# althonos/nafcodec

Measured on AMD Instinct MI355X. Metric: decoded Gbases/s (+ GB/s off HBM) at 1/2/4/8 MI355X vs CPU ref, higher is better.
Workload: dtype u8; 1 GPU; synthetic 10.0 GB DNA-only .naf (seq+len), 40000000000 bases, 73052 records, 152588 zstd blocks / 610352 Huffman streams in all, zstd-level-1 shape (L1), full-size check against the WRITER's checksums of bases and record table skipped

## Files before the change

nafcodec_amd/csrc/huf_flat.hip:

```cpp
#include <hip/hip_runtime.h>

#include <cstdlib>

#include "kernels.h"
#include "plan.h"

namespace nafgpu {

namespace {

#ifdef NAFGPU_EMU
#define NAFGPU_FLAT_INLINE inline
#else
#define NAFGPU_FLAT_INLINE __forceinline__
#endif

constexpr uint32_t kFlatThreads = 256;
constexpr uint32_t kFlatUnroll = 4;

__device__ inline void flat_flag_error(uint32_t *status, uint32_t code, uint32_t detail) {
    if (atomicCAS(&status[0], 0u, code) == 0u) status[1] = detail;
}

__device__ inline uint32_t flat_nib_char(uint32_t nib, uint32_t t_char) {
    const uint64_t lo = 0x425359434B47002Dull | (static_cast<uint64_t>(t_char) << 8);
    const uint64_t hi = 0x4E56484D44525741ull;
    return static_cast<uint32_t>(((nib & 8u) ? hi : lo) >> (8u * (nib & 7u))) & 0xFFu;
}
__device__ inline uint32_t flat_byte_chars(uint32_t b, uint32_t t_char) {
    return flat_nib_char(b & 15u, t_char) | (flat_nib_char(b >> 4, t_char) << 8);
}

template <bool ASCII, uint32_t L>
__device__ NAFGPU_FLAT_INLINE void flat_stream(const uint8_t *sp, uint32_t n, uint8_t *dp, const uint16_t *__restrict__ x1, uint32_t t_char,
                                   uint32_t *s_tbl) {
    constexpr uint32_t kOutB = ASCII ? 2 : 1;
    constexpr uint32_t kSyms = 16 / kOutB;
    constexpr uint32_t kPer = L <= 4 ? 2 : 1;
    constexpr uint32_t kIdxBits = kPer * L;
    constexpr uint32_t kLookB = kPer * kOutB;
    constexpr uint32_t kWords = (kSyms * L + 31) / 32;
    constexpr uint32_t kCodeMask = (1u << L) - 1u;
    const uint32_t tid = threadIdx.x;

    for (uint32_t i = tid; i < (1u << kIdxBits); i += kFlatThreads) {
        const uint32_t s1 = x1[kPer == 2 ? i >> L : i] & 0xFFu, s2 = x1[i & kCodeMask] & 0xFFu;
        const uint32_t o1 = ASCII ? flat_byte_chars(s1, t_char) : s1, o2 = ASCII ? flat_byte_chars(s2, t_char) : s2;
        s_tbl[i] = kPer == 2 ? o1 | (o2 << (8 * kOutB)) : o1;
    }
    __syncthreads();

    const uint32_t h = static_cast<uint32_t>(reinterpret_cast<uintptr_t>(dp) & 15u);
    uint8_t *const d16 = dp - h;
    const uintptr_t sa = reinterpret_cast<uintptr_t>(sp);
    const uint32_t *const sw = reinterpret_cast<const uint32_t *>(sp - (sa & 3u));
    const uint32_t sbit = static_cast<uint32_t>(sa & 3u) * 8u;
    const uint32_t end = h + n * kOutB;
    const uint32_t pf0 = h ? 1u : 0u, pf1 = end >> 4;
    constexpr uint32_t kStepWords = kFlatThreads * kSyms * L / 32u;
    uint32_t first = pf0 + tid;
    uint32_t r = 0;
    const uint32_t *w0 = sw;
    if (first < pf1) {
        const uint32_t lo = (n - (first * 16u - h) / kOutB - kSyms) * L + sbit;
        r = lo & 31u;
        w0 = sw + (lo >> 5);
    }
    auto load_round = [&](uint32_t p0, const uint32_t *w, uint32_t (&raw)[kFlatUnroll][kWords + 1]) {
#pragma unroll
        for (uint32_t u = 0; u < kFlatUnroll; u++) {
            const uint32_t *wu = p0 + u * kFlatThreads < pf1 ? w - u * kStepWords : w;
#pragma unroll
            for (uint32_t k = 0; k <= kWords; k++) raw[u][k] = wu[k];
        }
    };
    uint32_t cur[kFlatUnroll][kWords + 1];
    if (first < pf1) load_round(first, w0, cur);
    while (first < pf1) {
        const uint32_t next = first + kFlatUnroll * kFlatThreads;
        const uint32_t *w1 = w0 - kFlatUnroll * kStepWords;
        uint32_t nxt[kFlatUnroll][kWords + 1];
        if (next < pf1) load_round(next, w1, nxt);
#pragma unroll
        for (uint32_t u = 0; u < kFlatUnroll; u++) {
            const uint32_t p = first + u * kFlatThreads;
            uint32_t nw[kWords];
#pragma unroll
            for (uint32_t k = 0; k < kWords; k++) nw[k] = __builtin_amdgcn_alignbit(cur[u][k + 1], cur[u][k], r);
            uint32_t o[4] = {0, 0, 0, 0};
#pragma unroll
            for (uint32_t t = 0; t < kSyms / kPer; t++) {
                const uint32_t off = (kSyms - kPer * (t + 1u)) * L, q = off >> 5, s = off & 31u;
                uint32_t v = nw[q] >> s;
                if (s + kIdxBits > 32u) v |= nw[q + 1] << (32u - s);
                const uint32_t e = s_tbl[v & ((1u << kIdxBits) - 1u)];
                o[(t * kLookB) >> 2] |= e << (8u * ((t * kLookB) & 3u));
            }
            if (p < pf1) *reinterpret_cast<uint4 *>(d16 + static_cast<size_t>(p) * 16u) = make_uint4(o[0], o[1], o[2], o[3]);
        }
        if (next < pf1) {
#pragma unroll
            for (uint32_t u = 0; u < kFlatUnroll; u++)
#pragma unroll
                for (uint32_t k = 0; k <= kWords; k++) cur[u][k] = nxt[u][k];
        }
        first = next;
        w0 = w1;
    }
    const bool tail = (end & 15u) != 0 && (pf1 != 0 || !h);
    if ((tid == 0 && h) || (tid == 1 && tail)) {
        const uint32_t p = tid == 0 ? 0u : pf1;
        const int32_t j0 = (static_cast<int32_t>(p * 16u) - static_cast<int32_t>(h)) / static_cast<int32_t>(kOutB);
        for (uint32_t i = 0; i < kSyms; i++) {
            const int32_t j = j0 + static_cast<int32_t>(i);
            if (j < 0 || static_cast<uint32_t>(j) >= n) continue;
            const uint32_t b = (n - 1u - static_cast<uint32_t>(j)) * L;
            uint32_t v = sp[b >> 3];
            if ((b & 7u) + L > 8u) v |= static_cast<uint32_t>(sp[(b >> 3) + 1u]) << 8;
            const uint32_t code = (v >> (b & 7u)) & kCodeMask;
            const uint32_t e = s_tbl[kPer == 2 ? code << L : code];
            uint8_t *d = dp + static_cast<size_t>(j) * kOutB;
            d[0] = static_cast<uint8_t>(e);
            if (ASCII) d[1] = static_cast<uint8_t>(e >> 8);
        }
    }
}

template <bool ASCII>
__global__ __launch_bounds__(256) void k_huf_flat(const uint8_t *__restrict__ src, const HufTask *__restrict__ tasks,
                                                  const HufTblCopy *__restrict__ copies, const HufStream *__restrict__ streams,
                                                  const uint16_t *__restrict__ pool, const uint64_t *__restrict__ blk_base,
                                                  uint8_t *dst_base, uint32_t t_char, uint32_t *status) {
    constexpr uint32_t kOutB = ASCII ? 2 : 1;
    __shared__ uint32_t s_tbl[256];
    if (status[0] != 0) return;
    const HufTask task = tasks[blockIdx.x / static_cast<uint32_t>(kHufWave)];
    const uint32_t k = blockIdx.x % static_cast<uint32_t>(kHufWave);
    if (k >= task.n_streams) return;
    const uint32_t me = task.first_stream + k;
    const HufStream st = streams[me];
    const uint32_t L = st.max_bits;
    const uint32_t lastb = src[st.src_end - 1];
    const uint32_t hb = 31u - static_cast<uint32_t>(__clz(static_cast<int>(lastb | 1u)));
    const uint64_t bits = static_cast<uint64_t>(st.src_len - 1u) * 8u + hb;
    if (lastb == 0 || bits != static_cast<uint64_t>(st.n_syms) * L) {
        if (threadIdx.x == 0) flat_flag_error(status, kStHufBadEnd, me);
        return;
    }
    const uint8_t *sp = src + (st.src_end - st.src_len);
    uint8_t *dp = dst_base + ((st.flags & 1u) ? st.dst : (blk_base[st.blk] + static_cast<uint32_t>(st.dst)) * kOutB);
    const uint16_t *x1 = pool + copies[task.first_copy + st.tbl_lds].pool_off;
    switch (L) {
    case 1: flat_stream<ASCII, 1>(sp, st.n_syms, dp, x1, t_char, s_tbl); break;
    case 2: flat_stream<ASCII, 2>(sp, st.n_syms, dp, x1, t_char, s_tbl); break;
    case 3: flat_stream<ASCII, 3>(sp, st.n_syms, dp, x1, t_char, s_tbl); break;
    case 4: flat_stream<ASCII, 4>(sp, st.n_syms, dp, x1, t_char, s_tbl); break;
    case 5: flat_stream<ASCII, 5>(sp, st.n_syms, dp, x1, t_char, s_tbl); break;
    case 6: flat_stream<ASCII, 6>(sp, st.n_syms, dp, x1, t_char, s_tbl); break;
    case 7: flat_stream<ASCII, 7>(sp, st.n_syms, dp, x1, t_char, s_tbl); break;
    case 8: flat_stream<ASCII, 8>(sp, st.n_syms, dp, x1, t_char, s_tbl); break;
    default:
        if (threadIdx.x == 0) flat_flag_error(status, kStInternal, me);
        break;
    }
}

}

void launch_huf_flat(hipStream_t stream, const uint8_t *src, const HufTask *tasks, const HufClass &cls, const HufTblCopy *copies,
                     const HufStream *streams, const uint16_t *pool, const uint64_t *blk_base, uint8_t *out, uint8_t *lit,
                     bool ascii, uint32_t t_char, uint32_t *status) {
    if (!cls.n_tasks) return;
    const HufTask *t0 = tasks + cls.first_task;
    const dim3 grid(cls.n_tasks * static_cast<uint32_t>(kHufWave));
    if (ascii && !cls.to_lit)
        hipLaunchKernelGGL(k_huf_flat<true>, grid, dim3(kFlatThreads), 0, stream, src, t0, copies, streams, pool, blk_base, out, t_char, status);
    else
        hipLaunchKernelGGL(k_huf_flat<false>, grid, dim3(kFlatThreads), 0, stream, src, t0, copies, streams, pool, blk_base,
                           cls.to_lit ? lit : out, t_char, status);
}

}
```

Measured before the change: 4292 Gbases/s.

## Software-pipeline flat Huffman decode with ping-pong register rounds and early loads

Restructures the flat Huffman stream loop. Full rounds now run as unguarded double-buffered pairs: the next round's words are loaded while the current one is decoded and stored. Compiler barriers pin the load/store order, and the table staging into LDS is deferred until after the first loads are issued, so it overlaps with their latency. The kernel also hoists the status, pool-offset and block-base loads together and adds an occupancy hint to launch bounds. This trades extra register pressure and more code for better memory-latency hiding, with a guarded tail loop handling the remainder.

```diff
diff --git a/nafcodec_amd/csrc/huf_flat.hip b/nafcodec_amd/csrc/huf_flat.hip
--- a/nafcodec_amd/csrc/huf_flat.hip
+++ b/nafcodec_amd/csrc/huf_flat.hip
@@ -17,6 +17,8 @@
 
 constexpr uint32_t kFlatThreads = 256;
 constexpr uint32_t kFlatUnroll = 4;
+
+__device__ inline void flat_order() { asm volatile("" ::: "memory"); }
 
 __device__ inline void flat_flag_error(uint32_t *status, uint32_t code, uint32_t detail) {
     if (atomicCAS(&status[0], 0u, code) == 0u) status[1] = detail;
@@ -43,12 +45,14 @@
     constexpr uint32_t kCodeMask = (1u << L) - 1u;
     const uint32_t tid = threadIdx.x;
 
-    for (uint32_t i = tid; i < (1u << kIdxBits); i += kFlatThreads) {
-        const uint32_t s1 = x1[kPer == 2 ? i >> L : i] & 0xFFu, s2 = x1[i & kCodeMask] & 0xFFu;
-        const uint32_t o1 = ASCII ? flat_byte_chars(s1, t_char) : s1, o2 = ASCII ? flat_byte_chars(s2, t_char) : s2;
-        s_tbl[i] = kPer == 2 ? o1 | (o2 << (8 * kOutB)) : o1;
-    }
-    __syncthreads();
+    auto stage = [&]() {
+        for (uint32_t i = tid; i < (1u << kIdxBits); i += kFlatThreads) {
+            const uint32_t s1 = x1[kPer == 2 ? i >> L : i] & 0xFFu, s2 = x1[i & kCodeMask] & 0xFFu;
+            const uint32_t o1 = ASCII ? flat_byte_chars(s1, t_char) : s1, o2 = ASCII ? flat_byte_chars(s2, t_char) : s2;
+            s_tbl[i] = kPer == 2 ? o1 | (o2 << (8 * kOutB)) : o1;
+        }
+        __syncthreads();
+    };
 
     const uint32_t h = static_cast<uint32_t>(reinterpret_cast<uintptr_t>(dp) & 15u);
     uint8_t *const d16 = dp - h;
@@ -58,54 +62,85 @@
     const uint32_t end = h + n * kOutB;
     const uint32_t pf0 = h ? 1u : 0u, pf1 = end >> 4;
     constexpr uint32_t kStepWords = kFlatThreads * kSyms * L / 32u;
+    constexpr uint32_t kRound = kFlatUnroll * kFlatThreads;
     uint32_t first = pf0 + tid;
     uint32_t r = 0;
-    const uint32_t *w0 = sw;
+    uint32_t w0 = 0;
     if (first < pf1) {
         const uint32_t lo = (n - (first * 16u - h) / kOutB - kSyms) * L + sbit;
         r = lo & 31u;
-        w0 = sw + (lo >> 5);
-    }
-    auto load_round = [&](uint32_t p0, const uint32_t *w, uint32_t (&raw)[kFlatUnroll][kWords + 1]) {
-#pragma unroll
-        for (uint32_t u = 0; u < kFlatUnroll; u++) {
-            const uint32_t *wu = p0 + u * kFlatThreads < pf1 ? w - u * kStepWords : w;
+        w0 = lo >> 5;
+    }
+    auto words = [&](uint32_t w) { return reinterpret_cast<const uint32_t *>(reinterpret_cast<const uint8_t *>(sw) + w * 4u); };
+    auto piece = [&](uint32_t p) { return reinterpret_cast<uint4 *>(d16 + p * 16u); };
+    using Raw = uint32_t[kFlatUnroll][kWords + 1];
+    auto decode = [&](const uint32_t (&raw)[kWords + 1]) {
+        uint32_t nw[kWords];
+#pragma unroll
+        for (uint32_t k = 0; k < kWords; k++) nw[k] = __builtin_amdgcn_alignbit(raw[k + 1], raw[k], r);
+        uint32_t o[4] = {0, 0, 0, 0};
+#pragma unroll
+        for (uint32_t t = 0; t < kSyms / kPer; t++) {
+            const uint32_t off = (kSyms - kPer * (t + 1u)) * L, q = off >> 5, s = off & 31u;
+            uint32_t v = nw[q] >> s;
+            if (s + kIdxBits > 32u) v |= nw[q + 1] << (32u - s);
+            const uint32_t e = s_tbl[v & ((1u << kIdxBits) - 1u)];
+            o[(t * kLookB) >> 2] |= e << (8u * ((t * kLookB) & 3u));
+        }
+        return make_uint4(o[0], o[1], o[2], o[3]);
+    };
+    auto load_whole = [&](uint32_t w, Raw &raw) {
+#pragma unroll
+        for (uint32_t u = 0; u < kFlatUnroll; u++) {
+            const uint32_t *wu = words(w - u * kStepWords);
 #pragma unroll
             for (uint32_t k = 0; k <= kWords; k++) raw[u][k] = wu[k];
         }
-    };
-    uint32_t cur[kFlatUnroll][kWords + 1];
-    if (first < pf1) load_round(first, w0, cur);
-    while (first < pf1) {
-        const uint32_t next = first + kFlatUnroll * kFlatThreads;
-        const uint32_t *w1 = w0 - kFlatUnroll * kStepWords;
-        uint32_t nxt[kFlatUnroll][kWords + 1];
-        if (next < pf1) load_round(next, w1, nxt);
+        flat_order();
+    };
+    auto store_whole = [&](uint32_t p0, const Raw &raw) {
+#pragma unroll
+        for (uint32_t u = 0; u < kFlatUnroll; u++) {
+            *piece(p0 + u * kFlatThreads) = decode(raw[u]);
+            flat_order();
+        }
+    };
+    const uint32_t pairs = pf1 > pf0 ? (pf1 - pf0) / (2u * kRound) : 0u;
+    constexpr uint32_t kRoundWords = kFlatUnroll * kStepWords;
+    if (pairs) {
+        Raw a, b;
+        load_whole(w0, a);
+        load_whole(w0 - kRoundWords, b);
+        stage();
+        store_whole(first, a);
+        for (uint32_t i = 1; i < pairs; i++) {
+            load_whole(w0 - 2 * kRoundWords, a);
+            store_whole(first + kRound, b);
+            load_whole(w0 - 3 * kRoundWords, b);
+            store_whole(first + 2 * kRound, a);
+            first += 2 * kRound;
+            w0 -= 2 * kRoundWords;
+        }
+        store_whole(first + kRound, b);
+        first += 2 * kRound;
+        w0 -= 2 * kRoundWords;
+    } else {
+        stage();
+    }
+    for (; first < pf1; first += kRound, w0 -= kRoundWords) {
+        Raw c;
+#pragma unroll
+        for (uint32_t u = 0; u < kFlatUnroll; u++) {
+            const uint32_t *wu = words(first + u * kFlatThreads < pf1 ? w0 - u * kStepWords : w0);
+#pragma unroll
+            for (uint32_t k = 0; k <= kWords; k++) c[u][k] = wu[k];
+        }
 #pragma unroll
         for (uint32_t u = 0; u < kFlatUnroll; u++) {
             const uint32_t p = first + u * kFlatThreads;
-            uint32_t nw[kWords];
-#pragma unroll
-            for (uint32_t k = 0; k < kWords; k++) nw[k] = __builtin_amdgcn_alignbit(cur[u][k + 1], cur[u][k], r);
-            uint32_t o[4] = {0, 0, 0, 0};
-#pragma unroll
-            for (uint32_t t = 0; t < kSyms / kPer; t++) {
-                const uint32_t off = (kSyms - kPer * (t + 1u)) * L, q = off >> 5, s = off & 31u;
-                uint32_t v = nw[q] >> s;
-                if (s + kIdxBits > 32u) v |= nw[q + 1] << (32u - s);
-                const uint32_t e = s_tbl[v & ((1u << kIdxBits) - 1u)];
-                o[(t * kLookB) >> 2] |= e << (8u * ((t * kLookB) & 3u));
-            }
-            if (p < pf1) *reinterpret_cast<uint4 *>(d16 + static_cast<size_t>(p) * 16u) = make_uint4(o[0], o[1], o[2], o[3]);
-        }
-        if (next < pf1) {
-#pragma unroll
-            for (uint32_t u = 0; u < kFlatUnroll; u++)
-#pragma unroll
-                for (uint32_t k = 0; k <= kWords; k++) cur[u][k] = nxt[u][k];
-        }
-        first = next;
-        w0 = w1;
+            const uint4 o = decode(c[u]);
+            if (p < pf1) *piece(p) = o;
+        }
     }
     const bool tail = (end & 15u) != 0 && (pf1 != 0 || !h);
     if ((tid == 0 && h) || (tid == 1 && tail)) {
@@ -127,20 +162,24 @@
 }
 
 template <bool ASCII>
-__global__ __launch_bounds__(256) void k_huf_flat(const uint8_t *__restrict__ src, const HufTask *__restrict__ tasks,
+__global__ __launch_bounds__(256, ASCII ? 8 : 7) void k_huf_flat(const uint8_t *__restrict__ src, const HufTask *__restrict__ tasks,
                                                   const HufTblCopy *__restrict__ copies, const HufStream *__restrict__ streams,
                                                   const uint16_t *__restrict__ pool, const uint64_t *__restrict__ blk_base,
                                                   uint8_t *dst_base, uint32_t t_char, uint32_t *status) {
     constexpr uint32_t kOutB = ASCII ? 2 : 1;
     __shared__ uint32_t s_tbl[256];
-    if (status[0] != 0) return;
+    const uint32_t stopped = status[0];
     const HufTask task = tasks[blockIdx.x / static_cast<uint32_t>(kHufWave)];
     const uint32_t k = blockIdx.x % static_cast<uint32_t>(kHufWave);
-    if (k >= task.n_streams) return;
+    if (stopped != 0 || k >= task.n_streams) return;
     const uint32_t me = task.first_stream + k;
     const HufStream st = streams[me];
+    flat_order();
     const uint32_t L = st.max_bits;
     const uint32_t lastb = src[st.src_end - 1];
+    const uint32_t pool_off = copies[task.first_copy + st.tbl_lds].pool_off;
+    const uint64_t base = blk_base[st.blk];
+    flat_order();
     const uint32_t hb = 31u - static_cast<uint32_t>(__clz(static_cast<int>(lastb | 1u)));
     const uint64_t bits = static_cast<uint64_t>(st.src_len - 1u) * 8u + hb;
     if (lastb == 0 || bits != static_cast<uint64_t>(st.n_syms) * L) {
@@ -148,8 +187,8 @@
         return;
     }
     const uint8_t *sp = src + (st.src_end - st.src_len);
-    uint8_t *dp = dst_base + ((st.flags & 1u) ? st.dst : (blk_base[st.blk] + static_cast<uint32_t>(st.dst)) * kOutB);
-    const uint16_t *x1 = pool + copies[task.first_copy + st.tbl_lds].pool_off;
+    uint8_t *dp = dst_base + ((st.flags & 1u) ? st.dst : (base + static_cast<uint32_t>(st.dst)) * kOutB);
+    const uint16_t *x1 = pool + pool_off;
     switch (L) {
     case 1: flat_stream<ASCII, 1>(sp, st.n_syms, dp, x1, t_char, s_tbl); break;
     case 2: flat_stream<ASCII, 2>(sp, st.n_syms, dp, x1, t_char, s_tbl); break;
```

Result: faster. 4358 Gbases/s (median of 6 runs) (+1.5%).
